# pliam1105/BoxFusion

Measured on AMD Instinct MI355X. Metric: RGB-D frames/sec (whole node) on 640x480 stream, higher is better.
Workload: dtype bf16; 1 GPU; configs[2]: synthetic 640x480 RGB-D, batch 8/step/GPU, gap=1, CuTR ViT-B RGB-D + CLIP ViT-H/14 x16 crops/frame + fusion; frames=440, global_batch=8, parallelism=dp1, inflight_batches_per_gpu=2, scene_objects=30, fused_boxes=83, global_boxes=30

## Files before the change

### boxfusion_amd/_abi.py

```python
import ctypes
import functools
import os
import re

_INCLUDE = os.path.join(os.path.dirname(os.path.abspath(__file__)), "..", "include")
HEADER = os.path.join(_INCLUDE, "boxfusion_hip.h")
EXTENSION_HEADERS = (os.path.join(_INCLUDE, "boxfusion_objects.h"),)

_SCALAR = {"int": ctypes.c_int, "float": ctypes.c_float, "double": ctypes.c_double, "size_t": ctypes.c_size_t,
           "long long": ctypes.c_longlong, "int64_t": ctypes.c_int64, "int32_t": ctypes.c_int32}
_RETURN = {"int": ctypes.c_int, "size_t": ctypes.c_size_t, "const char*": ctypes.c_char_p, "void": None}


@functools.lru_cache(maxsize=None)
def _source(header=None):
    with open(header or HEADER) as f:
        return re.sub(r"/\*.*?\*/|//[^\n]*", " ", f.read(), flags=re.S)


def _ctype(decl, where, known, header=None):
    decl = " ".join(decl.split())
    if "*" in decl:
        return ctypes.c_void_p
    if decl not in known:
        raise TypeError(f"{header or HEADER}: {where}: no ctypes mapping for {decl!r}")
    return known[decl]


def struct(name, header=None):
    return _struct(name, header or HEADER)


@functools.lru_cache(maxsize=None)
def _struct(name, path):
    header = path
    body = re.search(r"typedef\s+struct\s*\{([^{}]*)\}\s*%s\s*;" % re.escape(name), _source(header))
    if body is None:
        raise KeyError(f"{path}: no typedef struct {name}")
    fields = []
    for decl in filter(None, (d.strip() for d in body.group(1).split(";"))):
# ... 79 lines not shown
```

### boxfusion_amd/_lib.py

```python
from __future__ import annotations

import atexit
import ctypes
import functools
import threading
import weakref
import sys
import os

import numpy as np
import torch

from . import _abi

HERE = os.path.dirname(os.path.abspath(__file__))
LIB_PATH = os.environ.get("BF_LIB_PATH") or os.path.join(HERE, "libboxfusion_hip.so")
_LIB = None

c_float, c_void_p = ctypes.c_float, ctypes.c_void_p

_C = _abi.constants()
BF_DEV_FUSION_LIST_OVERFLOW, BF_DEV_HULL_OVERFLOW, BF_DEV_VIEW_OVERFLOW, BF_DEV_INDEX_RANGE, BF_DEV_HULL_TRUNC = (
    _C["BF_DEV_" + n] for n in ("FUSION_LIST_OVERFLOW", "HULL_OVERFLOW", "VIEW_OVERFLOW", "INDEX_RANGE", "HULL_TRUNC"))
STATS_WORDS, ICP_ROW, ROWS_MAX_FIELDS, FSEQ_STATE_N = (
# ... 470 lines not shown
    _TLS.knobs = {**getattr(_TLS, "knobs", {}), **kw} if kw else {}


def _knobs():
    return getattr(_TLS, "knobs", {})


def _plan(plan):
    if plan is None:
        k = {f: v for f, v in _knobs().items() if f != "attn_variant"}
        b = cu_budget()
        if not b and not k:
            return None
        plan = GemmPlan(**{"cu_budget": b, **k})
    elif isinstance(plan, dict):
        plan = GemmPlan(**{"cu_budget": cu_budget(), **plan})
    return ctypes.byref(plan)


def gemm_tile_rows(M, N, K, plan=None):
    r = lib().bf_gemm_tile_rows_plan(M, N, K, _plan(plan))
    if r <= 0:
        raise HipError(f"bf_gemm_tile_rows_plan failed with bf_status {r}")
    return r


def gemm_grid(M, N, K, plan=None):
    r = lib().bf_gemm_grid_plan(M, N, K, _plan(plan))
    if r <= 0:
        raise HipError(f"bf_gemm_grid_plan failed with bf_status {r}")
    return r


def _gemm_work(a, w, bias=None, act=None, resid=None, resid_mod=0, out=None, out_dtype=torch.bfloat16,
               row_map=None, m=None, plan=None):
    M = a.shape[0] if m is None else m
    N, K = w.shape
    ob = (out.dtype if out is not None else out_dtype) == torch.bfloat16
    tags = dict(kind="gemm", act=ACT[act], out_bf16=ob, resid=resid is not None, M=M, N=N, K=K,
                large=bool(lib().bf_gemm_large_tiles(M, N, K)))
    nbytes = 2.0 * (M * K + N * K) + M * N * (2 if ob else 4)
    if resid is not None:
        nbytes += 4.0 * (M * N if not resid_mod else resid_mod * N)
    return tags, 2.0 * M * N * K, nbytes


@_timed(_gemm_work)
def gemm(a, w, bias=None, act=None, resid=None, resid_mod=0, out=None, out_dtype=torch.bfloat16,
         row_map=None, m=None, plan=None):
    _need(a, torch.bfloat16, "a")
    _need(w, torch.bfloat16, "w")
    M = a.shape[0] if m is None else m
    N, K = w.shape
    if out is None:
        out = torch.empty((M, N), dtype=out_dtype, device=a.device)
    c_bf16 = 1 if out.dtype == torch.bfloat16 else 0
    if not c_bf16 and out.dtype != torch.float32:
        raise HipError("gemm output must be bf16 or f32")
    if resid is not None:
        _need(resid, torch.float32, "resid")
    if bias is not None:
        _need(bias, torch.float32, "bias")
    if a.stride(1) != 1 or w.stride(1) != 1 or out.stride(1) != 1:
        raise HipError("gemm operands need unit column stride")
    _check(lib().bf_gemm_bf16_plan(a.data_ptr(), a.stride(0), w.data_ptr(), w.stride(0),
                                   _ptr(bias) if bias is not None else None,
# ... 1 lines not shown
                                   resid.stride(0) if resid is not None else 0, resid_mod,
                                   out.data_ptr(), out.stride(0), c_bf16,
                                   _ptr(row_map) if row_map is not None else None, M, N, K, ACT[act],
                                   _plan(plan), _stream()), "bf_gemm_bf16")
    return out


def _attention_work(q, k, v, o, batch, heads, sq, sk, head_dim, scale, q_bs=None, k_bs=None, v_bs=None,
                    o_bs=None, o_map=None, variant=0):
    bh = float(batch * heads)
    return (dict(kind="attn", D=head_dim, sq=sq, sk=sk, batch=batch, heads=heads),
            4.0 * bh * sq * sk * head_dim, 2.0 * bh * head_dim * (2 * sq + 2 * sk))


@_timed(_attention_work)
def attention(q, k, v, o, batch, heads, sq, sk, head_dim, scale, q_bs=None, k_bs=None, v_bs=None,
              o_bs=None, o_map=None, variant=0):
    for x, n in ((q, "q"), (k, "k"), (v, "v"), (o, "o")):
        _need(x, torch.bfloat16, n)
    q_bs = sq * q.stride(0) if q_bs is None else q_bs
    k_bs = sk * k.stride(0) if k_bs is None else k_bs
    v_bs = sk * v.stride(0) if v_bs is None else v_bs
    o_bs = sq * o.stride(0) if o_bs is None else o_bs
    if o_map is not None:
        _need(o_map, torch.int32, "o_map")
        if o_map.numel() < batch * sq:
            raise HipError(f"o_map has {o_map.numel()} rows < batch*sq = {batch * sq}")
    _check(lib().bf_attention_bf16_ex(q.data_ptr(), k.data_ptr(), v.data_ptr(), o.data_ptr(), batch,
                                      heads, sq, sk, head_dim, q.stride(0), k.stride(0),
                                      v.stride(0), o.stride(0), q_bs, k_bs, v_bs, o_bs, scale,
                                      _ptr(o_map) if o_map is not None else None,
                                      variant or _knobs().get("attn_variant", 0), _stream()),
           "bf_attention_bf16_ex")
    return o


def _attention_fp8out_work(q, k, v, o, batch, heads, sq, sk, head_dim, scale, out_qscale, q_bs=None,
                           k_bs=None, v_bs=None, o_bs=None, variant=0):
    bh = float(batch * heads)
    return (dict(kind="attn", D=head_dim, sq=sq, sk=sk, batch=batch, heads=heads, fp8out=True),
            4.0 * bh * sq * sk * head_dim, bh * head_dim * (2 * sq + 4 * sk + sq))


@_timed(_attention_fp8out_work)
def attention_fp8out(q, k, v, o, batch, heads, sq, sk, head_dim, scale, out_qscale, q_bs=None,
                     k_bs=None, v_bs=None, o_bs=None, variant=0):
    for x, n in ((q, "q"), (k, "k"), (v, "v")):
        _need(x, torch.bfloat16, n)
    _need(o, FP8, "o")
    q_bs = sq * q.stride(0) if q_bs is None else q_bs
    k_bs = sk * k.stride(0) if k_bs is None else k_bs
    v_bs = sk * v.stride(0) if v_bs is None else v_bs
    o_bs = sq * o.stride(0) if o_bs is None else o_bs
    _check(lib().bf_attention_fp8out_ex(q.data_ptr(), k.data_ptr(), v.data_ptr(), o.data_ptr(), batch, heads,
                                        sq, sk, head_dim, q.stride(0), k.stride(0), v.stride(0), o.stride(0),
                                        q_bs, k_bs, v_bs, o_bs, scale, out_qscale,
                                        variant or _knobs().get("attn_variant", 0), _stream()),
           "bf_attention_fp8out_ex")
    return o


def layernorm(x, weight, bias, eps, out=None, row_map=None, out_dtype=torch.bfloat16):
    _need(x, torch.float32, "x")
    M, C = x.shape
    if out is None:
        out = torch.empty((M, C), dtype=out_dtype, device=x.device)
# ... 1357 lines not shown
```

### boxfusion_amd/build.py

```python
from __future__ import annotations

import os
import subprocess
import sys
from concurrent.futures import ThreadPoolExecutor

HERE = os.path.dirname(os.path.abspath(__file__))
CSRC = os.path.join(HERE, "csrc")
BUILD = os.path.join(HERE, "_build")
LIB = os.path.join(HERE, "libboxfusion_hip.so")
ARCH = os.environ.get("BF_OFFLOAD_ARCH", "gfx950")

EXACT = ["-ffp-contract=off", "-fhip-fp32-correctly-rounded-divide-sqrt"]
SOURCES = {
    "bf_misc.hip": [],
    "bf_geom.hip": EXACT,
    "bf_depth.hip": EXACT,
    "bf_iou3d.hip": EXACT,
    "bf_assoc.hip": EXACT,
    "bf_fusion.hip": EXACT,
    "bf_dec_native.hip": EXACT,
    "bf_ingest.hip": EXACT,
    "bf_png.hip": EXACT,
    "bf_jpeg.hip": EXACT,
    "bf_fseq.hip": EXACT,
    "bf_cloud.hip": EXACT,
    "bf_eval.hip": EXACT,
    "bf_render.hip": EXACT,
    "bf_tsdf.hip": EXACT,
    "bf_track.hip": EXACT,
    "bf_fern.hip": EXACT,
    "bf_objects.hip": EXACT,
}
EXTRA = [s for s in sorted(os.listdir(CSRC)) if s.endswith(".hip") and s not in SOURCES]


def hipcc():
    for c in (os.environ.get("HIPCC"), "/opt/rocm/bin/hipcc", "hipcc"):
        if c and (os.path.isabs(c) and os.path.exists(c) or not os.path.isabs(c)):
            return c
    return "hipcc"


def _compile(src, flags):
    obj = os.path.join(BUILD, src.replace(".hip", ".o"))
    path = os.path.join(CSRC, src)
    deps = [path, os.path.join(CSRC, "bf_common.h"), os.path.join(CSRC, "bf_cv2.h"), os.path.join(CSRC, "bf_compact.h"),
            os.path.join(HERE, "..", "include", "boxfusion_hip.h"),
            os.path.join(HERE, "..", "include", "boxfusion_objects.h")]
    if os.path.exists(obj) and all(os.path.getmtime(obj) >= os.path.getmtime(d) for d in deps
                                   if os.path.exists(d)):
        return obj
    cmd = [hipcc(), f"--offload-arch={ARCH}", "-O3", "-fPIC", "-std=c++17", "-c", path, "-o", obj,
           "-Wno-unused-result"] + flags
    r = subprocess.run(cmd, capture_output=True, text=True)
    if r.returncode != 0:
        raise RuntimeError(f"hipcc failed for {src}:\n{r.stderr}")
    return obj


def build(verbose=False) -> str:
    os.makedirs(BUILD, exist_ok=True)
    jobs = dict(SOURCES)
    for s in EXTRA:
        jobs[s] = []
    with ThreadPoolExecutor(max_workers=min(8, len(jobs))) as ex:
        objs = list(ex.map(lambda kv: _compile(*kv), jobs.items()))
    if not os.path.exists(LIB) or any(os.path.getmtime(o) > os.path.getmtime(LIB) for o in objs):
        cmd = [hipcc(), f"--offload-arch={ARCH}", "-shared", "-fPIC", "-o", LIB] + objs
        r = subprocess.run(cmd, capture_output=True, text=True)
        if r.returncode != 0:
            raise RuntimeError(f"link failed:\n{r.stderr}")
    if verbose:
        print(LIB)
    return LIB


if __name__ == "__main__":
    build(verbose=True)
    sys.exit(0)
```

### boxfusion_amd/csrc/bf_attn.hip

```cpp
#include "bf_common.h"

#include <type_traits>
#include <climits>
#include <algorithm>

typedef __bf16 bf16x8 __attribute__((ext_vector_type(8)));
typedef float f32x16 __attribute__((ext_vector_type(16)));
typedef unsigned short u16;

#define AT_THREADS 256
#define AT_QT 128
#define AT_KT 64

struct alignas(16) V128 {
    uint32_t x, y, z, w;
};
struct alignas(8) V64 {
    uint32_t x, y;
};

__device__ __forceinline__ u16 at_f2bf(float f) {
    __bf16 b = (__bf16)f;
    return *reinterpret_cast<u16*>(&b);
}

__device__ __forceinline__ long long attn_out_offset(const int32_t* __restrict__ o_map, int b, int q,
                                                     int sq, long long o_bs, int o_rs) {
    if (!o_map) return b * o_bs + (long long)q * o_rs;
    if (q >= sq) return -1;
    const int r = o_map[(long long)b * sq + q];
    return r < 0 ? -1 : (long long)r * o_rs;
}

// ... 48 lines not shown
        const float m_new = fmaxf(m_run, mt);
        const float alpha = __builtin_amdgcn_exp2f(m_run - m_new);
        m_run = m_new;
        l_run *= alpha;
#pragma unroll
        for (int db = 0; db < DB; ++db)
#pragma unroll
            for (int e = 0; e < 16; ++e) o[db][e] *= alpha;
    }
    float ls = 0.f;
#pragma unroll
    for (int sub = 0; sub < 2; ++sub) {
        if (sub == 1 && !sub1) {
#pragma unroll
            for (int e = 0; e < 16; ++e) pf[1][e >> 3][e & 7] = (__bf16)0.0f;
            continue;
        }
#pragma unroll
        for (int e = 0; e < 16; ++e) {
            const float p = __builtin_amdgcn_exp2f(fmaf(s[sub][e], c, -m_run));
            if (!ONES) ls += p;
            pf[sub][e >> 3][e & 7] = (__bf16)p;
        }
    }
    if (!ONES) l_run += ls;
}

#ifndef ATTN_WPE64
#define ATTN_WPE64 3
#endif
#ifndef ATTN_WPE80
#define ATTN_WPE80 3
#endif
template <int D, int NW, bool F8O = false, bool CAUSAL = false, bool LSTQ = false>
__global__ void __launch_bounds__(NW * 64, (D == 64 && NW == 4) ? ATTN_WPE64 : (D == 80 && NW == 4 && !CAUSAL) ? ATTN_WPE80 : 1)
k_attn2(const u16* __restrict__ Q, const u16* __restrict__ K,
                                                      const u16* __restrict__ V, u16* __restrict__ O,
                                                      int sq, int sk, int q_rs, int k_rs, int v_rs,
                                                      int o_rs, long long q_bs, long long k_bs,
                                                      long long v_bs, long long o_bs, float scale_log2,
                                                      const int32_t* __restrict__ o_map, float oqs = 1.f) {
    constexpr int KS = D / 16;
    constexpr int DB = (D + 31) / 32;
    constexpr bool ONES = (D % 32) != 0;
    constexpr int KROW = D + 8;
    constexpr int VROW = attn_vrow_bytes(D) / 2;
    constexpr int KTILE = AT_KT * KROW;
    constexpr int VTILE = AT_KT * VROW;
    constexpr int CPR = D / 8;
    constexpr int CH = AT_KT * CPR;
    constexpr int NT = NW * 64;
    constexpr int NBUF = 2;
    __shared__ __attribute__((aligned(16))) u16 sK[NBUF * KTILE];
    __shared__ __attribute__((aligned(16))) u16 sV[NBUF * VTILE];
    constexpr bool LST = LSTQ && !CAUSAL && D % 16 == 0;
    constexpr int EB = F8O ? 1 : 2;
    constexpr int OROW = ((EB * D + 16) / 32) * 32 + 16;
    constexpr bool OWN = NW >= 8;
    static_assert(!LST || OWN || NW * 32 * OROW <= NBUF * KTILE * 2, "staged rows fit the K ring");
    __shared__ __attribute__((aligned(16))) unsigned char sO[LST && OWN ? NW * 32 * OROW : 16];

    const int t = threadIdx.x, lane = t & 63, wave = t >> 6;
    const AttnBlk blk = attn_block(1);
    const int h = blk.h, b = blk.b;
    const int fr = lane & 31, fh = lane >> 5;
    const int q = blk.qb * (NW * 32) + wave * 32 + fr;
    const bool idle = blk.qb * (NW * 32) + wave * 32 >= sq;
    const u16* Qb = Q + b * q_bs + h * D;
    const u16* Kb = K + b * k_bs + h * D;
    const u16* Vb = V + b * v_bs + h * D;

    bf16x8 qf[KS];
#pragma unroll
    for (int ks = 0; ks < KS; ++ks)
        qf[ks] = *reinterpret_cast<const bf16x8*>(Qb + (size_t)min(q, sq - 1) * q_rs + 16 * ks + 8 * fh);
    if (VROW > D)
        for (int i = t; i < NBUF * AT_KT * (VROW - D); i += NT) {
            const int r = i / (VROW - D), c = i % (VROW - D);
            sV[r * VROW + D + c] = (ONES && c == 0) ? (u16)0x3F80 : (u16)0;
        }

    static_assert(CH % 64 == 0 && NT % 64 == 0, "wave-uniform staging guard");
    constexpr int NTS = NT;
    const int ts = t;
    constexpr int NSO = (CH + NTS - 1) / NTS;
    typedef unsigned u32x4 __attribute__((ext_vector_type(4)));
    u32x4 stk[NSO], stv[NSO];
    int srow[NSO], scol[NSO];
#pragma unroll
    for (int i = 0; i < NSO; ++i) {
        const int c = min(ts + i * NTS, CH - 1);
        srow[i] = c / CPR;
        scol[i] = (c % CPR) * 8;
    }
    auto stage_load = [&](int k0_) {
#pragma unroll
        for (int i = 0; i < NSO; ++i) {
            const int key = min(k0_ + srow[i], sk - 1);
            stk[i] = *reinterpret_cast<const u32x4*>(Kb + (size_t)key * k_rs + scol[i]);
            stv[i] = *reinterpret_cast<const u32x4*>(Vb + (size_t)key * v_rs + scol[i]);
        }
    };
    auto stage_store = [&](int buf_) {
#pragma unroll
        for (int i = 0; i < NSO; ++i) {
            if (ts + i * NTS < CH) {
                *reinterpret_cast<u32x4*>(sK + buf_ * KTILE + srow[i] * KROW + scol[i]) = stk[i];
                *reinterpret_cast<u32x4*>(sV + buf_ * VTILE + srow[i] * VROW + scol[i]) = stv[i];
            }
        }
    };

    f32x16 o[DB];
#pragma unroll
    for (int db = 0; db < DB; ++db)
#pragma unroll
        for (int e = 0; e < 16; ++e) o[db][e] = 0.f;
    float m_run = -INFINITY, l_run = 0.f;
    const int g16 = (lane >> 4) & 1, q4 = (lane & 15) >> 2, p4 = lane & 3;
    const int ntiles = (sk + AT_KT - 1) / AT_KT;
    const int nfull = sk / AT_KT;

    auto qk = [&](int tile, f32x16 (&s)[2], bool maybe_tail) {
        const int k0 = tile * AT_KT;
        const u16* kt = sK + (tile % NBUF) * KTILE;
        const bool sub1 = !maybe_tail || (k0 + 32 < sk);
#pragma unroll
        for (int sub = 0; sub < 2; ++sub) {
// ... 82 lines not shown
        if (idle) return;
        unsigned char* wreg = (OWN ? sO : reinterpret_cast<unsigned char*>(sK)) + wave * 32 * OROW;
#pragma unroll
        for (int db = 0; db < DB; ++db)
#pragma unroll
            for (int g = 0; g < 4; ++g) {
                const int d0 = db * 32 + 8 * g + 4 * fh;
                if (d0 >= D) continue;
                if constexpr (F8O) {
                    const float sc = inv * oqs;
                    float a[4];
#pragma unroll
                    for (int i = 0; i < 4; ++i) a[i] = fminf(fmaxf(o[db][4 * g + i] * sc, -448.f), 448.f);
                    int pk = __builtin_amdgcn_cvt_pk_fp8_f32(a[0], a[1], 0, false);
                    pk = __builtin_amdgcn_cvt_pk_fp8_f32(a[2], a[3], pk, true);
                    *reinterpret_cast<int*>(wreg + fr * OROW + d0) = pk;
                } else {
                    V64 w;
                    w.x = (uint32_t)at_f2bf(o[db][4 * g + 0] * inv) | ((uint32_t)at_f2bf(o[db][4 * g + 1] * inv) << 16);
                    w.y = (uint32_t)at_f2bf(o[db][4 * g + 2] * inv) | ((uint32_t)at_f2bf(o[db][4 * g + 3] * inv) << 16);
                    *reinterpret_cast<V64*>(wreg + fr * OROW + 2 * d0) = w;
                }
            }
        constexpr int CPRO = EB * D / 16;
        unsigned char* Ob = reinterpret_cast<unsigned char*>(O);
#pragma unroll
        for (int j = 0; j < (32 * CPRO + 63) / 64; ++j) {
            const int c = lane + 64 * j;
            if (c >= 32 * CPRO) break;
            const int r = c / CPRO, col = c % CPRO;
            const int qr = q - fr + r;
            const V128 val = *reinterpret_cast<const V128*>(wreg + r * OROW + 16 * col);
            const long long off = attn_out_offset(o_map, b, qr, sq, o_bs, o_rs);
            if (qr < sq && off >= 0) *reinterpret_cast<V128*>(Ob + EB * (off + h * D) + 16 * col) = val;
        }
        return;
    }
    const long long o_off = attn_out_offset(o_map, b, q, sq, o_bs, o_rs);
    if (q < sq && o_off >= 0) {
        const float inv = 1.0f / l;
        if constexpr (F8O) {
            unsigned char* orow = reinterpret_cast<unsigned char*>(O) + o_off + h * D;
            const float sc = inv * oqs;
#pragma unroll
            for (int db = 0; db < DB; ++db)
#pragma unroll
                for (int g = 0; g < 4; ++g) {
                    const int d0 = db * 32 + 8 * g + 4 * fh;
                    if (d0 >= D) continue;
                    float a[4];
#pragma unroll
                    for (int i = 0; i < 4; ++i) a[i] = fminf(fmaxf(o[db][4 * g + i] * sc, -448.f), 448.f);
                    int pk = __builtin_amdgcn_cvt_pk_fp8_f32(a[0], a[1], 0, false);
                    pk = __builtin_amdgcn_cvt_pk_fp8_f32(a[2], a[3], pk, true);
                    *reinterpret_cast<int*>(orow + d0) = pk;
                }
        } else {
            u16* orow = O + o_off + h * D;
#pragma unroll
            for (int db = 0; db < DB; ++db)
#pragma unroll
                for (int g = 0; g < 4; ++g) {
                    const int d0 = db * 32 + 8 * g + 4 * fh;
                    if (d0 >= D) continue;
                    V64 w;
                    w.x = (uint32_t)at_f2bf(o[db][4 * g + 0] * inv) | ((uint32_t)at_f2bf(o[db][4 * g + 1] * inv) << 16);
                    w.y = (uint32_t)at_f2bf(o[db][4 * g + 2] * inv) | ((uint32_t)at_f2bf(o[db][4 * g + 3] * inv) << 16);
                    *reinterpret_cast<V64*>(orow + d0) = w;
                }
        }
    }
}
// ... 25 lines not shown
    if (nw_one <= 2) { LAUNCH_2(DD, 2, false); }                                                  \
    else if (eight) { if (lst) { LAUNCH_2(DD, 8, true); } else { LAUNCH_2(DD, 8, false); } }      \
    else if (nine) { if (lst) { LAUNCH_2(DD, 9, true); } else { LAUNCH_2(DD, 9, false); } }       \
    else if (wide8) { if (lst) { LAUNCH_2(DD, 8, true); } else { LAUNCH_2(DD, 8, false); } }      \
    else { if (lst) { LAUNCH_2(DD, 4, true); } else { LAUNCH_2(DD, 4, false); } }
    switch (head_dim) {
        case 32: LAUNCH_2D(32); break;
        case 64: LAUNCH_2D(64); break;
        case 80: LAUNCH_2D(80); break;
        case 128: LAUNCH_2(128, 4, false); break;
        default: return BF_ERR_UNSUPPORTED;
    }
#undef LAUNCH_2D
#undef LAUNCH_2
    return bf_check_launch();
}

BF_API int bf_attention_bf16_omap(const void* q, const void* k, const void* v, void* o, int batch,
                                  int heads, int sq, int sk, int head_dim, int q_rs, int k_rs,
                                  int v_rs, int o_rs, long long q_bs, long long k_bs, long long v_bs,
                                  long long o_bs, float scale, const int32_t* o_map, void* stream) {
    return bf_attention_bf16_ex(q, k, v, o, batch, heads, sq, sk, head_dim, q_rs, k_rs, v_rs, o_rs, q_bs, k_bs,
                                v_bs, o_bs, scale, o_map, 0, stream);
}

BF_API int bf_attention_bf16(const void* q, const void* k, const void* v, void* o, int batch,
                             int heads, int sq, int sk, int head_dim, int q_rs, int k_rs, int v_rs,
                             int o_rs, long long q_bs, long long k_bs, long long v_bs,
                             long long o_bs, float scale, void* stream) {
    return bf_attention_bf16_omap(q, k, v, o, batch, heads, sq, sk, head_dim, q_rs, k_rs, v_rs, o_rs,
                                  q_bs, k_bs, v_bs, o_bs, scale, nullptr, stream);
}

BF_API int bf_attention_fp8out_ex(const void* q, const void* k, const void* v, void* o, int batch,
                                  int heads, int sq, int sk, int head_dim, int q_rs, int k_rs, int v_rs,
                                  int o_rs, long long q_bs, long long k_bs, long long v_bs, long long o_bs,
                                  float scale, float out_qscale, int variant, void* stream) {
    const int av = variant == 0 ? 6 : variant;
    if (!q || !k || !v || !o || batch <= 0 || heads <= 0 || sq <= 0 || sk <= 0 || !(out_qscale > 0.f))
        return BF_ERR_ARG;
    if ((q_rs | k_rs | v_rs) % 8 != 0 || o_rs % 4 != 0 || o_bs % 4 != 0) return BF_ERR_UNSUPPORTED;
    const float sl2 = scale * 1.4426950408889634f;
    const int nw_one = (sq + 31) / 32;
    const bool lst = av != 27;
    const hipStream_t st = bf_stream(stream);
#define LAUNCH_8(DD, NWV, LS)                                                                     \
    hipLaunchKernelGGL((k_attn2<DD, NWV, true, false, LS>), dim3((sq + NWV * 32 - 1) / (NWV * 32), heads, batch), \
                       dim3(NWV * 64), 0, st, (const u16*)q, (const u16*)k, (const u16*)v, (u16*)o, sq, sk, \
                       q_rs, k_rs, v_rs, o_rs, q_bs, k_bs, v_bs, o_bs, sl2, (const int32_t*)nullptr, out_qscale)
    const bool nine = nw_one > 4 && nw_one <= 9 && !(head_dim == 80 && nw_one == 9 && av != 28);
#define LAUNCH_8D(DD)                                                                             \
    if (nine) { if (lst) { LAUNCH_8(DD, 9, true); } else { LAUNCH_8(DD, 9, false); } }             \
    else { if (lst) { LAUNCH_8(DD, 4, true); } else { LAUNCH_8(DD, 4, false); } }
    switch (head_dim) {
        case 64: LAUNCH_8D(64); break;
        case 80: LAUNCH_8D(80); break;
        default: return BF_ERR_UNSUPPORTED;
    }
#undef LAUNCH_8D
#undef LAUNCH_8
    return bf_check_launch();
}

BF_API int bf_attention_fp8out(const void* q, const void* k, const void* v, void* o, int batch,
                               int heads, int sq, int sk, int head_dim, int q_rs, int k_rs, int v_rs,
                               int o_rs, long long q_bs, long long k_bs, long long v_bs, long long o_bs,
// ... 24 lines not shown
```

### boxfusion_amd/csrc/bf_gemm.hip

```cpp
#include "bf_common.h"

#include <mutex>
#include <set>
#include <string>

#ifndef GEMM_PRIO_MODE
#define GEMM_PRIO_MODE 0
#endif

#ifndef GEMM_TILE_FIXED
#define GEMM_TILE_FIXED 0.7
#endif

#ifndef GEMM_TACC
#define GEMM_TACC 0
#endif

typedef __bf16 bf16x8 __attribute__((ext_vector_type(8)));
typedef float f32x16 __attribute__((ext_vector_type(16)));
typedef float f32x4 __attribute__((ext_vector_type(4)));
typedef unsigned short u16;

#define GB_M 128
#define GB_N 128
#define GB_K 64
#define G_THREADS 256

struct alignas(16) U128 {
    uint32_t x, y, z, w;
};

__device__ __forceinline__ float bf2f(u16 v) { return __uint_as_float(((uint32_t)v) << 16); }
__device__ __forceinline__ u16 f2bf(float f) {
// ... 1271 lines not shown
                              const int32_t* row_map, int M, int N, int K) {
    static bool attr = false;
    if (!attr) {
        hipFuncSetAttribute((const void*)k_gemm_skinny<OB, AC>, hipFuncAttributeMaxDynamicSharedMemorySize, SK_LDS);
        attr = true;
    }
    hipLaunchKernelGGL((k_gemm_skinny<OB, AC>), dim3(N / 32, (M + 127) / 128), dim3(SK_THREADS), SK_LDS,
                       bf_stream(stream), (const u16*)A, lda, (const u16*)W, ldw, bias, resid, ldr, resid_mod, C,
                       ldc, row_map, M, N, K);
    return bf_check_launch();
}

static bool gemm_log_on() {
    static const bool on = [] { const char* e = getenv("BF_GEMM_LOG"); return e && e[0] == '1'; }();
    return on;
}

static void gemm_log_line(const char* line) {
    static std::mutex& mu = *new std::mutex;
    static std::set<std::string>& seen = *new std::set<std::string>;
    std::lock_guard<std::mutex> g(mu);
    if (seen.insert(line).second) fprintf(stderr, "%s\n", line);
}

static void gemm_log(int M, int N, int K, int act, int resid, int resid_mod, int row_map, int c_bf16,
                     const char* kern, int bm) {
    if (!gemm_log_on()) return;
    char buf[256];
    snprintf(buf, sizeof buf, "bf_gemm M=%d N=%d K=%d act=%d resid=%d resid_mod=%d row_map=%d out=%s -> %s rows=%d",
             M, N, K, act, resid, resid_mod, row_map, c_bf16 ? "bf16" : "f32", kern, bm);
    gemm_log_line(buf);
}

static void gemm_log_fp8(int M, int N, int K, int act, int resid, int out_kind, const char* kern, int bm) {
    if (!gemm_log_on()) return;
    char buf[256];
    snprintf(buf, sizeof buf, "bf_gemm_fp8 M=%d N=%d K=%d act=%d resid=%d out=%s -> %s rows=%d", M, N, K, act, resid,
             out_kind == 0 ? "f32" : out_kind == 1 ? "bf16" : "fp8", kern, bm);
    gemm_log_line(buf);
}

BF_API int bf_gemm_bf16_plan(const void* A, int lda, const void* W, int ldw, const float* bias,
                             const float* resid, int ldr, int resid_mod, void* C, int ldc, int c_bf16,
                             const int32_t* row_map, int M, int N, int K, int act, const bf_gemm_plan* plan,
                             void* stream) {
    const GemmCfg cfg = gemm_cfg(plan);
    if (!A || !W || !C || M < 0 || N <= 0 || K <= 0) return BF_ERR_ARG;
    if (K % GB_K != 0 || lda % 8 != 0 || ldw % 8 != 0) return BF_ERR_UNSUPPORTED;
    if (M == 0) return BF_OK;
    if ((long long)(M - 1) * lda * 2 + (long long)K * 2 >= (1LL << 31) ||
        (long long)(N - 1) * ldw * 2 + (long long)K * 2 >= (1LL << 31))
        return BF_ERR_CAPACITY;
    const int tiles_m = (M + GB_M - 1) / GB_M, tiles_n = (N + GB_N - 1) / GB_N;
    const int nwg = tiles_m * tiles_n;
    const size_t lds = 2 * 32768;
    if (act < 0 || act > 2) return BF_ERR_ARG;
    const int cw = c_bf16 ? 8 : 4;
    const int vec_epi = (N % cw == 0) && ((uintptr_t)C % 16 == 0) && ((size_t)ldc * (c_bf16 ? 2 : 4) % 16 == 0) &&
                        (!resid || (((uintptr_t)resid % 16 == 0) && (ldr % 4 == 0)));
    const int t2m = (M + 255) / 256, t2n = (N + 255) / 256;
    const long long t2 = (long long)t2m * t2n;
    if (gemm_use_skinny(M, N, K, vec_epi && (c_bf16 || N % 8 == 0), cfg)) {
        gemm_log(M, N, K, act, resid != nullptr, resid_mod, row_map != nullptr, c_bf16, "k_gemm_skinny", 128);
#define GSK(OB, AC) return launch_gemm_skinny<OB, AC>(stream, A, lda, W, ldw, bias, resid, ldr, resid_mod, C, ldc, \
                                                      row_map, M, N, K)
        if (c_bf16) {
// ... 142 lines not shown
```

### boxfusion_amd/engine.py

```python
from __future__ import annotations

import math
import os

import numpy as np
import torch
import torch.nn.functional as F

from boxfusion_amd import _lib
from boxfusion_amd.clip import CLIP_MEAN, CLIP_STD
from boxfusion_amd.cubify_transformer import FrameBatch
from boxfusion_amd.preprocessor import PIXEL_MEAN, PIXEL_STD
from boxfusion_amd.vit import get_abs_pos


def _bf(w):
    return w.detach().to(torch.bfloat16).contiguous()


def _f(w):
    return w.detach().to(torch.float32).contiguous()


class CuTREngine:

    def __init__(self, model, batch, height=480, width=640, pad=640, device="cuda", depth_ratio=1,
                 native_decoder=None):
        dev = torch.device(device)
        if native_decoder is None:
            native_decoder = os.environ.get("BF_DECODER_TORCH", "0") != "1"
        self.native_decoder = bool(native_decoder)
        self.decoder = None
        self.model = model.to(dev).eval()
        vit = model.backbone.backbone
        self.dev, self.B, self.H, self.W, self.P = dev, batch, height, width, pad
        self.C, self.heads = vit.embed_dim, vit.num_heads
        self.D = self.C // self.heads
        p = vit.patch_size
        if pad % p or height > pad or width > pad:
            raise ValueError(f"frame {height}x{width} does not fit the {pad} square")
        self.g = pad // p
        self.ws = vit.window_size
        self.nwx = math.ceil(self.g / self.ws)
        self.nw = self.nwx * self.nwx
        self.T = self.g * self.g
        self.has_depth = bool(vit.depth_modality)
        if self.has_depth:
            r = int(depth_ratio)
            if r not in (1, 2, 4) or pad % (p * r) or self.ws % r:
                raise ValueError(f"unsupported rgb -> depth ratio {depth_ratio} for pad {pad}")
            self.r = r
            self.Pd = pad // r
            self.gd = self.g // r
            self.wsd = self.ws // r
            if math.ceil(self.gd / self.wsd) != self.nwx:
                raise ValueError("depth windows do not pair with the RGB windows")
            self.Td = self.gd * self.gd
        else:
            self.r, self.Pd, self.gd, self.wsd, self.Td = None, 0, 0, 0, 0
        self.win_rgb = self.ws * self.ws
        self.win_rows = self.win_rgb + self.wsd * self.wsd
# ... 3 lines not shown
        with torch.no_grad():
            self.pos = _f(get_abs_pos(vit.pos_embed, vit.pretrain_use_cls_token, (self.g, self.g)).reshape(T, C))
            if self.has_depth:
                self.patchd_w = _bf(vit.patch_embed_depth.proj.weight.reshape(C, -1))
                self.patchd_b = _f(vit.patch_embed_depth.proj.bias)
                self.posd = _f(get_abs_pos(vit.pos_embed_depth, vit.pretrain_use_cls_token,
                                           (self.gd, self.gd)).reshape(Td, C))
        self.blocks = []
        for blk in vit.blocks:
            proj_w, proj_b = blk.attn.proj.weight, blk.attn.proj.bias
            fc2_w, fc2_b = blk.mlp.fc2.weight, blk.mlp.fc2.bias
            with torch.no_grad():
                if blk.ls1 is not None:
                    proj_w, proj_b = blk.ls1.gamma[:, None] * proj_w, blk.ls1.gamma * proj_b
                if blk.ls2 is not None:
                    fc2_w, fc2_b = blk.ls2.gamma[:, None] * fc2_w, blk.ls2.gamma * fc2_b
            self.blocks.append(dict(
                window=blk.window_size > 0, depth=bool(blk.depth_modality) and self.has_depth,
                n1=(_f(blk.norm1.weight), _f(blk.norm1.bias), blk.norm1.eps),
                n2=(_f(blk.norm2.weight), _f(blk.norm2.bias), blk.norm2.eps),
                qkv=(_bf(blk.attn.qkv.weight), _f(blk.attn.qkv.bias)),
                proj=(_bf(proj_w), _f(proj_b)),
                fc1=(_bf(blk.mlp.fc1.weight), _f(blk.mlp.fc1.bias)),
                fc2=(_bf(fc2_w), _f(fc2_b))))
        en = vit.encoder_norm
        self.enc_norm = None if isinstance(en, torch.nn.Identity) else (_f(en.weight), _f(en.bias), en.eps)
        depth_blocks = [i for i, b in enumerate(self.blocks) if b["depth"]]
        self.last_depth = max(depth_blocks) if depth_blocks else -1
        bf16, f32 = dict(dtype=torch.bfloat16, device=dev), dict(dtype=torch.float32, device=dev)
        nwr = B * self.nw * self.win_rows
        rows = B * T + B * Td
        self.rows = rows
        self.X = torch.zeros((rows, C), **f32)
        self.LNW = torch.zeros((nwr, C), **bf16)
        self.QKV = torch.empty((max(nwr, B * T), 3 * C), **bf16)
        self.ATT = torch.zeros((rows, C), **bf16)
        self.LN2 = torch.empty((rows, C), **bf16)
        self.H1 = torch.empty((rows, 4 * C), **bf16)
        self.A_rgb = torch.empty((B * T, 3 * p * p), **bf16)
        self.A_d = torch.empty((B * Td, p * p), **bf16) if self.has_depth else None
        self.OUT = torch.empty((B * T, C), **f32) if self.enc_norm is not None else None
        self.win_in, self.win_out = self._window_maps()
        if self.win_out is not None:
            w = self.win_out.view(B * self.nw, self.win_rows).clone()
            self.win_out_rgbq = w[:, :self.win_rgb].contiguous().view(-1)
        self._pos_cache = {}

    def _window_maps(self):
        B, T, g, ws, nwx = self.B, self.T, self.g, self.ws, self.nwx
        b, y, x = np.meshgrid(np.arange(B), np.arange(g), np.arange(g), indexing="ij")
        w = (y // ws) * nwx + (x // ws)
        win_in = [((b * self.nw + w) * self.win_rows + (y % ws) * ws + (x % ws)).reshape(-1)]
        xrow = [(b * T + y * g + x).reshape(-1)]
        if self.has_depth:
            gd, wsd = self.gd, self.wsd
            b, y, x = np.meshgrid(np.arange(B), np.arange(gd), np.arange(gd), indexing="ij")
            w = (y // wsd) * nwx + (x // wsd)
            win_in.append(((b * self.nw + w) * self.win_rows + self.win_rgb + (y % wsd) * wsd + (x % wsd)).reshape(-1))
            xrow.append((B * T + b * self.Td + y * gd + x).reshape(-1))
        win_in, xrow = np.concatenate(win_in), np.concatenate(xrow)
        win_out = -np.ones(B * self.nw * self.win_rows, np.int64)
        win_out[win_in] = xrow
        to = lambda a: torch.as_tensor(a.astype(np.int32), device=self.dev)
        order = np.argsort(xrow)
        return to(win_in[order]), to(win_out)

    def backbone(self, img_u8, depth_std, chw=False, pixel_mean=PIXEL_MEAN, pixel_std=PIXEL_STD):
        B, T, C = self.B, self.T, self.C
        X = self.X
        Xr = X[: B * T]
        _lib.im2col_rgb8(img_u8, self.P, 16, pixel_mean, pixel_std, out=self.A_rgb, chw=chw)
        _lib.gemm(self.A_rgb, self.patch_w, self.patch_b, resid=self.pos, resid_mod=T, out=Xr)
        if self.has_depth:
            _lib.im2col_f32(depth_std, self.Pd, 16, out=self.A_d)
            _lib.gemm(self.A_d, self.patchd_w, self.patchd_b, resid=self.posd, resid_mod=self.Td,
                      out=X[B * T:])
        scale = self.D ** -0.5
        nb = B * self.nw
        for i, blk in enumerate(self.blocks):
            g1, b1, e1 = blk["n1"]
            g2, b2, e2 = blk["n2"]
            if blk["window"]:
                joint = blk["depth"]
                last = joint and i == self.last_depth
                src = X if joint else Xr
                _lib.layernorm(src, g1, b1, e1, out=self.LNW, row_map=self.win_in[: src.shape[0]])
                _lib.gemm(self.LNW, *blk["qkv"], out=self.QKV[: self.LNW.shape[0]])
                q = self.QKV[:, :C]
                rs = self.win_rows * self.QKV.stride(0)
                sq = self.win_rgb if (last or not joint) else self.win_rows
                _lib.attention(q, self.QKV[:, C:2 * C], self.QKV[:, 2 * C:], self.ATT, nb, self.heads,
                               sq, self.win_rows if joint else self.win_rgb, self.D, scale,
                               q_bs=rs, k_bs=rs, v_bs=rs, o_bs=0,
                               o_map=self.win_out_rgbq if sq == self.win_rgb and self.has_depth
                               else self.win_out)
                rows = B * T if (last or not joint) else self.rows
                Xm = X[:rows]
                _lib.gemm(self.ATT[:rows], *blk["proj"], resid=Xm, out=Xm)
            else:
                _lib.layernorm(Xr, g1, b1, e1, out=self.LN2[: B * T])
                qkv = self.QKV[: B * T]
                _lib.gemm(self.LN2[: B * T], *blk["qkv"], out=qkv)
                att = self.ATT[: B * T]
                _lib.attention(qkv[:, :C], qkv[:, C:2 * C], qkv[:, 2 * C:], att, B, self.heads, T, T,
                               self.D, scale)
                _lib.gemm(att, *blk["proj"], resid=Xr, out=Xr)
                rows = B * T
                Xm = Xr
            _lib.layernorm(Xm, g2, b2, e2, out=self.LN2[:rows])
            _lib.gemm(self.LN2[:rows], *blk["fc1"], act="gelu", out=self.H1[:rows])
            _lib.gemm(self.H1[:rows], *blk["fc2"], resid=Xm, out=Xm)
        out = Xr
        if self.enc_norm is not None:
            out = _lib.layernorm(Xr, self.enc_norm[0], self.enc_norm[1], self.enc_norm[2], out=self.OUT)
        return out.view(B, self.g, self.g, C).permute(0, 3, 1, 2)

    def ray_embedding(self, K_host, size_wh):
        K_host = np.asarray(K_host, np.float32)
        key = (tuple(K_host.reshape(-1).tolist()), tuple(size_wh))
        if key not in self._pos_cache:
            with torch.no_grad():
                K = torch.from_numpy(K_host).to(self.dev)
                self._pos_cache[key] = self.model.pos_embedding(K[None], [size_wh], self.g)[0]
        return self._pos_cache[key]

    def positions(self, K_host, image_sizes):
        key = (np.asarray(K_host, np.float32).tobytes(), tuple(image_sizes))
        if key not in self._pos_cache:
# ... 199 lines not shown
```

Before: 156.6 frames/s.

## Gather window tokens inside attention instead of padding windowed QKV buffers

Windowed attention blocks no longer scatter LayerNorm output into a padded per-window layout. LayerNorm and the QKV GEMM now run over the dense token rows, with one extra zero row for padding slots. A new gather variant of the attention kernel reads K/V and Q rows through index maps and skips query tiles that hold only padding. The QKV GEMM plan is pinned to the kernel class the padded shape would have used. This removes GEMM work on padding rows at the cost of indirect, less coalesced loads in attention.

```diff
diff --git a/boxfusion_amd/_abi.py b/boxfusion_amd/_abi.py
--- a/boxfusion_amd/_abi.py
+++ b/boxfusion_amd/_abi.py
@@ -5,7 +5,8 @@
 
 _INCLUDE = os.path.join(os.path.dirname(os.path.abspath(__file__)), "..", "include")
 HEADER = os.path.join(_INCLUDE, "boxfusion_hip.h")
-EXTENSION_HEADERS = (os.path.join(_INCLUDE, "boxfusion_objects.h"),)
+EXTENSION_HEADERS = (os.path.join(_INCLUDE, "boxfusion_objects.h"),
+                     os.path.join(_INCLUDE, "boxfusion_windows.h"))
 
 _SCALAR = {"int": ctypes.c_int, "float": ctypes.c_float, "double": ctypes.c_double, "size_t": ctypes.c_size_t,
            "long long": ctypes.c_longlong, "int64_t": ctypes.c_int64, "int32_t": ctypes.c_int32}
diff --git a/boxfusion_amd/_lib.py b/boxfusion_amd/_lib.py
--- a/boxfusion_amd/_lib.py
+++ b/boxfusion_amd/_lib.py
@@ -526,6 +526,13 @@
     return r
 
 
+def gemm_kernel_class(M, N, K):
+    r = lib().bf_gemm_bf16_kernel_class(M, N, K)
+    if r < 0:
+        raise HipError(f"bf_gemm_bf16_kernel_class failed with bf_status {r}")
+    return r
+
+
 def _gemm_work(a, w, bias=None, act=None, resid=None, resid_mod=0, out=None, out_dtype=torch.bfloat16,
                row_map=None, m=None, plan=None):
     M = a.shape[0] if m is None else m
@@ -593,6 +600,31 @@
                                       _ptr(o_map) if o_map is not None else None,
                                       variant or _knobs().get("attn_variant", 0), _stream()),
            "bf_attention_bf16_ex")
+    return o
+
+
+def _attention_gather_work(q, k, v, o, batch, heads, sq, sk, head_dim, scale, kv_map, q_map, q_cnt, o_map,
+                           n_rows=None):
+    bh = float(batch * heads)
+    return (dict(kind="attn", D=head_dim, sq=sq, sk=sk, batch=batch, heads=heads, gather=True),
+            4.0 * bh * sq * sk * head_dim, 2.0 * bh * head_dim * (2 * sq + 2 * sk))
+
+
+@_timed(_attention_gather_work)
+def attention_gather(q, k, v, o, batch, heads, sq, sk, head_dim, scale, kv_map, q_map, q_cnt, o_map,
+                     n_rows=None):
+    for x, n in ((q, "q"), (k, "k"), (v, "v"), (o, "o")):
+        _need(x, torch.bfloat16, n)
+    for m, n, size in ((kv_map, "kv_map", batch * sk), (q_map, "q_map", batch * sq), (q_cnt, "q_cnt", batch),
+                       (o_map, "o_map", batch * sq)):
+        _need(m, torch.int32, n)
+        if m.numel() < size:
+            raise HipError(f"{n} has {m.numel()} entries < {size}")
+    n_rows = min(q.shape[0], k.shape[0], v.shape[0]) if n_rows is None else n_rows
+    _check(lib().bf_attention_bf16_gather(q.data_ptr(), k.data_ptr(), v.data_ptr(), o.data_ptr(), batch, heads,
+                                          sq, sk, head_dim, q.stride(0), k.stride(0), v.stride(0), o.stride(0),
+                                          n_rows, scale, _ptr(kv_map), _ptr(q_map), _ptr(q_cnt), _ptr(o_map),
+                                          _stream()), "bf_attention_bf16_gather")
     return o
 
 
diff --git a/boxfusion_amd/build.py b/boxfusion_amd/build.py
--- a/boxfusion_amd/build.py
+++ b/boxfusion_amd/build.py
@@ -47,7 +47,8 @@
     path = os.path.join(CSRC, src)
     deps = [path, os.path.join(CSRC, "bf_common.h"), os.path.join(CSRC, "bf_cv2.h"), os.path.join(CSRC, "bf_compact.h"),
             os.path.join(HERE, "..", "include", "boxfusion_hip.h"),
-            os.path.join(HERE, "..", "include", "boxfusion_objects.h")]
+            os.path.join(HERE, "..", "include", "boxfusion_objects.h"),
+            os.path.join(HERE, "..", "include", "boxfusion_windows.h")]
     if os.path.exists(obj) and all(os.path.getmtime(obj) >= os.path.getmtime(d) for d in deps
                                    if os.path.exists(d)):
         return obj
diff --git a/boxfusion_amd/csrc/bf_attn.hip b/boxfusion_amd/csrc/bf_attn.hip
--- a/boxfusion_amd/csrc/bf_attn.hip
+++ b/boxfusion_amd/csrc/bf_attn.hip
@@ -1,4 +1,5 @@
 #include "bf_common.h"
+#include "../../include/boxfusion_windows.h"
 
 #include <type_traits>
 #include <climits>
@@ -113,14 +114,26 @@
 #ifndef ATTN_WPE80
 #define ATTN_WPE80 3
 #endif
-template <int D, int NW, bool F8O = false, bool CAUSAL = false, bool LSTQ = false>
+template <bool GATHER>
+struct AttnGather {};
+template <>
+struct AttnGather<true> {
+    const int32_t *kv_map, *q_map, *q_cnt;
+    int n_rows;
+};
+__device__ __forceinline__ unsigned attn_gather_row(const int32_t* __restrict__ map, long long i, int n_rows) {
+    return min((unsigned)map[i], (unsigned)(n_rows - 1));
+}
+
+template <int D, int NW, bool F8O = false, bool CAUSAL = false, bool LSTQ = false, bool GATHER = false>
 __global__ void __launch_bounds__(NW * 64, (D == 64 && NW == 4) ? ATTN_WPE64 : (D == 80 && NW == 4 && !CAUSAL) ? ATTN_WPE80 : 1)
 k_attn2(const u16* __restrict__ Q, const u16* __restrict__ K,
                                                       const u16* __restrict__ V, u16* __restrict__ O,
                                                       int sq, int sk, int q_rs, int k_rs, int v_rs,
                                                       int o_rs, long long q_bs, long long k_bs,
                                                       long long v_bs, long long o_bs, float scale_log2,
-                                                      const int32_t* __restrict__ o_map, float oqs = 1.f) {
+                                                      const int32_t* __restrict__ o_map, float oqs = 1.f,
+                                                      AttnGather<GATHER> ga = {}) {
     constexpr int KS = D / 16;
     constexpr int DB = (D + 31) / 32;
     constexpr bool ONES = (D % 32) != 0;
@@ -146,15 +159,27 @@
     const int h = blk.h, b = blk.b;
     const int fr = lane & 31, fh = lane >> 5;
     const int q = blk.qb * (NW * 32) + wave * 32 + fr;
-    const bool idle = blk.qb * (NW * 32) + wave * 32 >= sq;
+    int sqb = sq;
+    if constexpr (GATHER) {
+        sqb = min(ga.q_cnt[b], sq);
+        if (blk.qb * (NW * 32) >= sqb) return;
+    }
+    const bool idle = blk.qb * (NW * 32) + wave * 32 >= sqb;
     const u16* Qb = Q + b * q_bs + h * D;
     const u16* Kb = K + b * k_bs + h * D;
     const u16* Vb = V + b * v_bs + h * D;
 
     bf16x8 qf[KS];
-#pragma unroll
-    for (int ks = 0; ks < KS; ++ks)
-        qf[ks] = *reinterpret_cast<const bf16x8*>(Qb + (size_t)min(q, sq - 1) * q_rs + 16 * ks + 8 * fh);
+    if constexpr (GATHER) {
+        const size_t qrow = attn_gather_row(ga.q_map, (long long)b * sq + min(q, sqb - 1), ga.n_rows);
+#pragma unroll
+        for (int ks = 0; ks < KS; ++ks)
+            qf[ks] = *reinterpret_cast<const bf16x8*>(Qb + qrow * q_rs + 16 * ks + 8 * fh);
+    } else {
+#pragma unroll
+        for (int ks = 0; ks < KS; ++ks)
+            qf[ks] = *reinterpret_cast<const bf16x8*>(Qb + (size_t)min(q, sq - 1) * q_rs + 16 * ks + 8 * fh);
+    }
     if (VROW > D)
         for (int i = t; i < NBUF * AT_KT * (VROW - D); i += NT) {
             const int r = i / (VROW - D), c = i % (VROW - D);
@@ -174,7 +199,24 @@
         srow[i] = c / CPR;
         scol[i] = (c % CPR) * 8;
     }
+    unsigned krow[GATHER ? NSO : 1];
+    auto map_load = [&](int k0_) {
+#pragma unroll
+        for (int i = 0; i < NSO; ++i)
+            if constexpr (GATHER)
+                krow[i] = attn_gather_row(ga.kv_map, (long long)b * sk + min(k0_ + srow[i], sk - 1), ga.n_rows);
+    };
+    if constexpr (GATHER) map_load(0);
     auto stage_load = [&](int k0_) {
+        if constexpr (GATHER) {
+#pragma unroll
+            for (int i = 0; i < NSO; ++i) {
+                stk[i] = *reinterpret_cast<const u32x4*>(Kb + (size_t)krow[i] * k_rs + scol[i]);
+                stv[i] = *reinterpret_cast<const u32x4*>(Vb + (size_t)krow[i] * v_rs + scol[i]);
+            }
+            map_load(k0_ + AT_KT);
+            return;
+        }
 #pragma unroll
         for (int i = 0; i < NSO; ++i) {
             const int key = min(k0_ + srow[i], sk - 1);
@@ -323,12 +365,12 @@
             const int qr = q - fr + r;
             const V128 val = *reinterpret_cast<const V128*>(wreg + r * OROW + 16 * col);
             const long long off = attn_out_offset(o_map, b, qr, sq, o_bs, o_rs);
-            if (qr < sq && off >= 0) *reinterpret_cast<V128*>(Ob + EB * (off + h * D) + 16 * col) = val;
+            if (qr < sqb && off >= 0) *reinterpret_cast<V128*>(Ob + EB * (off + h * D) + 16 * col) = val;
         }
         return;
     }
     const long long o_off = attn_out_offset(o_map, b, q, sq, o_bs, o_rs);
-    if (q < sq && o_off >= 0) {
+    if (q < sqb && o_off >= 0) {
         const float inv = 1.0f / l;
         if constexpr (F8O) {
             unsigned char* orow = reinterpret_cast<unsigned char*>(O) + o_off + h * D;
@@ -420,6 +462,27 @@
                                   q_bs, k_bs, v_bs, o_bs, scale, nullptr, stream);
 }
 
+BF_API int bf_attention_bf16_gather(const void* q, const void* k, const void* v, void* o, int batch, int heads,
+                                    int sq, int sk, int head_dim, int q_rs, int k_rs, int v_rs, int o_rs,
+                                    int n_rows, float scale, const int32_t* kv_map, const int32_t* q_map,
+                                    const int32_t* q_cnt, const int32_t* o_map, void* stream) {
+    if (!q || !k || !v || !o || !kv_map || !q_map || !q_cnt || !o_map || batch <= 0 || heads <= 0 || sq <= 0 ||
+        sk <= 0 || n_rows <= 0)
+        return BF_ERR_ARG;
+    if (head_dim != 64 || (q_rs | k_rs | v_rs) % 8 != 0 || o_rs % 4 != 0) return BF_ERR_UNSUPPORTED;
+    const float sl2 = scale * 1.4426950408889634f;
+    const hipStream_t st = bf_stream(stream);
+    const AttnGather<true> ga{kv_map, q_map, q_cnt, n_rows};
+#define LAUNCH_G(NWV)                                                                             \
+    hipLaunchKernelGGL((k_attn2<64, NWV, false, false, true, true>), dim3((sq + NWV * 32 - 1) / (NWV * 32), heads, batch), \
+                       dim3(NWV * 64), 0, st, (const u16*)q, (const u16*)k, (const u16*)v, (u16*)o, sq, sk, q_rs, \
+                       k_rs, v_rs, o_rs, 0LL, 0LL, 0LL, 0LL, sl2, o_map, 1.f, ga)
+    if (sq > 448 && sq <= 512) { LAUNCH_G(8); }
+    else { LAUNCH_G(4); }
+#undef LAUNCH_G
+    return bf_check_launch();
+}
+
 BF_API int bf_attention_fp8out_ex(const void* q, const void* k, const void* v, void* o, int batch,
                                   int heads, int sq, int sk, int head_dim, int q_rs, int k_rs, int v_rs,
                                   int o_rs, long long q_bs, long long k_bs, long long v_bs, long long o_bs,
diff --git a/boxfusion_amd/csrc/bf_gemm.hip b/boxfusion_amd/csrc/bf_gemm.hip
--- a/boxfusion_amd/csrc/bf_gemm.hip
+++ b/boxfusion_amd/csrc/bf_gemm.hip
@@ -1,4 +1,5 @@
 #include "bf_common.h"
+#include "../../include/boxfusion_windows.h"
 
 #include <mutex>
 #include <set>
@@ -1336,6 +1337,13 @@
     gemm_log_line(buf);
 }
 
+BF_API int bf_gemm_bf16_kernel_class(int M, int N, int K) {
+    if (M <= 0 || N <= 0 || K <= 0) return BF_ERR_ARG;
+    const GemmCfg cfg = gemm_cfg(nullptr);
+    if (gemm_use_skinny(M, N, K, N % 8 == 0, cfg)) return 0;
+    return (N % 8 == 0 && gemm_use_large(M, N, K, cfg)) ? 2 : 1;
+}
+
 static void gemm_log_fp8(int M, int N, int K, int act, int resid, int out_kind, const char* kern, int bm) {
     if (!gemm_log_on()) return;
     char buf[256];
diff --git a/boxfusion_amd/engine.py b/boxfusion_amd/engine.py
--- a/boxfusion_amd/engine.py
+++ b/boxfusion_amd/engine.py
@@ -22,11 +22,35 @@
     return w.detach().to(torch.float32).contiguous()
 
 
+def window_gather_maps(slot_row, nq, sk, zero_row=0, shift=1):
+    slot_row = np.asarray(slot_row)[:, :sk]
+    W = slot_row.shape[0]
+    kv = np.where(slot_row < 0, zero_row, slot_row + shift)
+    ng = -(-nq // 32)
+    stride = 32 * ng
+    q_map = np.full((W, stride), zero_row, np.int64)
+    o_map = -np.ones((W, stride), np.int64)
+    q_cnt = np.zeros(W, np.int64)
+    for w in range(W):
+        j = 0
+        for s0 in range(0, nq, 32):
+            s1 = min(nq, s0 + 32)
+            if (slot_row[w, s0:s1] >= 0).any():
+                q_map[w, j:j + s1 - s0] = kv[w, s0:s1]
+                o_map[w, j:j + s1 - s0] = slot_row[w, s0:s1]
+                j += s1 - s0
+        q_cnt[w] = j
+    i32 = lambda a: np.ascontiguousarray(a.reshape(-1).astype(np.int32))
+    return i32(kv), i32(q_map), i32(q_cnt), i32(o_map), stride
+
+
 class CuTREngine:
 
     def __init__(self, model, batch, height=480, width=640, pad=640, device="cuda", depth_ratio=1,
-                 native_decoder=None):
+                 native_decoder=None, window_layout="gather"):
         dev = torch.device(device)
+        if window_layout not in ("gather", "padded"):
+            raise ValueError(f"window_layout {window_layout!r}: 'gather' or 'padded'")
         if native_decoder is None:
             native_decoder = os.environ.get("BF_DECODER_TORCH", "0") != "1"
         self.native_decoder = bool(native_decoder)
@@ -96,8 +120,14 @@
         rows = B * T + B * Td
         self.rows = rows
         self.X = torch.zeros((rows, C), **f32)
-        self.LNW = torch.zeros((nwr, C), **bf16)
-        self.QKV = torch.empty((max(nwr, B * T), 3 * C), **bf16)
+        self.window_layout = window_layout if self.D == 64 else "padded"
+        if self.window_layout == "gather":
+            self.LNW = None
+            self.LNT = torch.zeros((rows + 1, C), **bf16)
+            self.QKV = torch.empty((rows + 1, 3 * C), **bf16)
+        else:
+            self.LNW = torch.zeros((nwr, C), **bf16)
+            self.QKV = torch.empty((max(nwr, B * T), 3 * C), **bf16)
         self.ATT = torch.zeros((rows, C), **bf16)
         self.LN2 = torch.empty((rows, C), **bf16)
         self.H1 = torch.empty((rows, 4 * C), **bf16)
@@ -108,6 +138,20 @@
         if self.win_out is not None:
             w = self.win_out.view(B * self.nw, self.win_rows).clone()
             self.win_out_rgbq = w[:, :self.win_rgb].contiguous().view(-1)
+        if self.window_layout == "gather":
+            slot_row = self.win_out.view(B * self.nw, self.win_rows).cpu().numpy()
+            kinds = {"rgb": (self.win_rgb, self.win_rgb)}
+            if self.has_depth:
+                kinds.update(joint=(self.win_rows, self.win_rows), rgbq=(self.win_rgb, self.win_rows))
+            self.win_gather = {}
+            for kind, (nq, sk) in kinds.items():
+                *maps, stride = window_gather_maps(slot_row, nq, sk)
+                self.win_gather[kind] = tuple(torch.as_tensor(m, device=dev) for m in maps) + (stride, sk)
+            want = _lib.gemm_kernel_class(nwr, 3 * C, C)
+            self.qkv_plan = {}
+            for n in {rows + 1, B * T + 1}:
+                same = want == 0 or _lib.gemm_kernel_class(n, 3 * C, C) == want
+                self.qkv_plan[n] = None if same else {"kernel": 1 if want == 1 else -1}
         self._pos_cache = {}
 
     def _window_maps(self):
@@ -148,16 +192,26 @@
                 joint = blk["depth"]
                 last = joint and i == self.last_depth
                 src = X if joint else Xr
-                _lib.layernorm(src, g1, b1, e1, out=self.LNW, row_map=self.win_in[: src.shape[0]])
-                _lib.gemm(self.LNW, *blk["qkv"], out=self.QKV[: self.LNW.shape[0]])
-                q = self.QKV[:, :C]
-                rs = self.win_rows * self.QKV.stride(0)
-                sq = self.win_rgb if (last or not joint) else self.win_rows
-                _lib.attention(q, self.QKV[:, C:2 * C], self.QKV[:, 2 * C:], self.ATT, nb, self.heads,
-                               sq, self.win_rows if joint else self.win_rgb, self.D, scale,
-                               q_bs=rs, k_bs=rs, v_bs=rs, o_bs=0,
-                               o_map=self.win_out_rgbq if sq == self.win_rgb and self.has_depth
-                               else self.win_out)
+                if self.window_layout == "gather":
+                    n = src.shape[0]
+                    _lib.layernorm(src, g1, b1, e1, out=self.LNT[1:n + 1])
+                    qkv = self.QKV[:n + 1]
+                    _lib.gemm(self.LNT[:n + 1], *blk["qkv"], out=qkv, plan=self.qkv_plan[n + 1])
+                    kv_map, q_map, q_cnt, o_map, sq, sk = self.win_gather[
+                        "rgb" if not joint else "rgbq" if last else "joint"]
+                    _lib.attention_gather(qkv[:, :C], qkv[:, C:2 * C], qkv[:, 2 * C:], self.ATT, nb,
+                                          self.heads, sq, sk, self.D, scale, kv_map, q_map, q_cnt, o_map)
+                else:
+                    _lib.layernorm(src, g1, b1, e1, out=self.LNW, row_map=self.win_in[: src.shape[0]])
+                    _lib.gemm(self.LNW, *blk["qkv"], out=self.QKV[: self.LNW.shape[0]])
+                    q = self.QKV[:, :C]
+                    rs = self.win_rows * self.QKV.stride(0)
+                    sq = self.win_rgb if (last or not joint) else self.win_rows
+                    _lib.attention(q, self.QKV[:, C:2 * C], self.QKV[:, 2 * C:], self.ATT, nb, self.heads,
+                                   sq, self.win_rows if joint else self.win_rgb, self.D, scale,
+                                   q_bs=rs, k_bs=rs, v_bs=rs, o_bs=0,
+                                   o_map=self.win_out_rgbq if sq == self.win_rgb and self.has_depth
+                                   else self.win_out)
                 rows = B * T if (last or not joint) else self.rows
                 Xm = X[:rows]
                 _lib.gemm(self.ATT[:rows], *blk["proj"], resid=Xm, out=Xm)
diff --git a/include/boxfusion_windows.h b/include/boxfusion_windows.h
--- /dev/null
+++ b/include/boxfusion_windows.h
@@ -0,0 +1,21 @@
+#ifndef BOXFUSION_WINDOWS_H
+#define BOXFUSION_WINDOWS_H
+
+#include "boxfusion_hip.h"
+
+#ifdef __cplusplus
+extern "C" {
+#endif
+
+int bf_attention_bf16_gather(const void* q, const void* k, const void* v, void* o, int batch, int heads,
+                             int sq, int sk, int head_dim, int q_rs, int k_rs, int v_rs, int o_rs,
+                             int n_rows, float scale, const int32_t* kv_map, const int32_t* q_map,
+                             const int32_t* q_cnt, const int32_t* o_map, void* stream);
+
+int bf_gemm_bf16_kernel_class(int M, int N, int K);
+
+#ifdef __cplusplus
+}
+#endif
+
+#endif
```

New measurement: 157.5 frames/s (median of 6 runs). No clear change (+0.6%).
